# 42jaylonw/shifu

Hardware: AMD Instinct MI355X
Metric: env-steps/sec (whole node), A1 12-dof 4096 envs/GPU (higher is better)
Workload: dtype f32

## Files before the change

### shifu_amd/csrc/shf_a1_chain.hip

```cpp
#include <hip/hip_runtime.h>

#include "shf_chain.h"
#include "shf_chain_hard.h"

template <int G, bool TW, bool SELF = false>
__global__ __launch_bounds__(256, (G == 32 ? 2 : 1)) void k_a1_chain(A1Args A) { a1_chain_step_body<G, A1Chain, TW, SELF>(A); }

template <bool TW, bool SELF>
__global__ __launch_bounds__(256, 2) void k_a1_chain_pgs(A1Args A) { a1_chain_step_body<32, A1Chain, TW, SELF, true>(A); }
template <bool TW, bool SELF>
__global__ __launch_bounds__(256, 2) void k_a1_chain_pgs16(A1Args A) { a1_chain_step_body<32, A1Chain, TW, SELF, true, 16>(A); }
template <bool TW, bool SELF>
__global__ __launch_bounds__(256, 2) void k_a1_chain_tgs(A1Args A) { a1_chain_step_body<32, A1Chain, TW, SELF, true, 8, true>(A); }
template <bool TW, bool SELF>
__global__ __launch_bounds__(256, 2) void k_a1_chain_tgs16(A1Args A) { a1_chain_step_body<32, A1Chain, TW, SELF, true, 16, true>(A); }
#define SHF_PICK4(K, warped, self) ((self) ? ((warped) ? reinterpret_cast<const void*>(K<true, true>) : reinterpret_cast<const void*>(K<false, true>)) \
                                           : ((warped) ? reinterpret_cast<const void*>(K<true, false>) : reinterpret_cast<const void*>(K<false, false>)))
const void* shf_a1_chain_pgs_kernel(bool warped, bool self, bool k16, bool tgs) {
  if (tgs) return k16 ? SHF_PICK4(k_a1_chain_tgs16, warped, self) : SHF_PICK4(k_a1_chain_tgs, warped, self);
  return k16 ? SHF_PICK4(k_a1_chain_pgs16, warped, self) : SHF_PICK4(k_a1_chain_pgs, warped, self);
}
int shf_a1_chain_pgs_max_contacts(void) { return 16; }

template <bool TW, bool SELF, int KC, bool TGS>
DEV void sim_step_chain_pgs_body(const SimArgs& A) {
  extern __shared__ __attribute__((aligned(16))) float smem[];
  typedef A1Chain CD;
  constexpr int G = 32, nb = CD::NB, nd = CD::ND, NR = (CD::NEV + G - 1) / G;
  const int es = threadIdx.x / G, l = threadIdx.x % G;
  const int e = blockIdx.x * (256 / G) + es;
  stage_block<CHAIN_MODEL_BYTES>(A.model, smem);
  __syncthreads();
  const ShfModel* m = reinterpret_cast<const ShfModel*>(smem);
  if (e >= A.n) return;
  ChainLds L = chain_lds_carve<CD>(smem + CHAIN_MODEL_WORDS + es * chain_lds_words<CD>(0, SELF));
  const float* dof = A.dof + (size_t)e * nd * 2;
  const float* root = A.root + (size_t)e * 13;
  for (int i = l; i < 2 * nd; i += G) L.dofb[(i >> 1) * DOF_STRIDE + (i & 1)] = dof[i];
  if (l < 13) L.root[l] = root[l];
  GROUP_SYNC();
  StepCtx C;
  C.m = m; C.sp = A.sp; C.terr.t = A.terr; C.terr.h = A.heights; C.scene = nullptr;
  C.dropped = env_dropped(A.dropped, A.sp, e);
  C.mscale = A.mscale ? A.mscale + (size_t)e * nb : nullptr;
  const float mu = A.friction ? A.friction[e] : 1.0f;
  const int dl = l < nd ? l : 0;
  DofLane X = {L.dofb[dl * DOF_STRIDE], L.dofb[dl * DOF_STRIDE + 1], (A.effort && l < nd) ? A.effort[(size_t)e * nd + l] : 0.0f,
               (A.pos_tgt && l < nd) ? A.pos_tgt[(size_t)e * nd + l] : 0.0f, (A.vel_tgt && l < nd) ? A.vel_tgt[(size_t)e * nd + l] : 0.0f};
  ChainPoints<NR> LP;
  chain_points_load<G>(m, CD::NEV, l, C.sp.contact_offset + C.sp.rest_offset, LP);
  const RowLane RL = row_lane_load<CD>(l);
  chain_substep_hard<G, CD, TW, SELF, KC, TGS>(C, L, l, X, LP, RL, A.body_force ? A.body_force + (size_t)e * nb * 3 : nullptr, mu, L.xch);
  if (l < nd) {
    A.dof[((size_t)e * nd + l) * 2] = X.q;
    A.dof[((size_t)e * nd + l) * 2 + 1] = X.qd;
  }
  if (l < 13) A.root[(size_t)e * 13 + l] = L.root[l];
  for (int i = l; i < 3 * nb; i += G) A.contact[(size_t)e * nb * 3 + i] = L.xch[i];
}
template <bool TW, bool SELF>
__global__ __launch_bounds__(256, 2) void k_sim_step_chain_pgs(SimArgs A) { sim_step_chain_pgs_body<TW, SELF, 8, false>(A); }
template <bool TW, bool SELF>
__global__ __launch_bounds__(256, 2) void k_sim_step_chain_pgs16(SimArgs A) { sim_step_chain_pgs_body<TW, SELF, 16, false>(A); }
template <bool TW, bool SELF>
__global__ __launch_bounds__(256, 2) void k_sim_step_chain_tgs(SimArgs A) { sim_step_chain_pgs_body<TW, SELF, 8, true>(A); }
template <bool TW, bool SELF>
__global__ __launch_bounds__(256, 2) void k_sim_step_chain_tgs16(SimArgs A) { sim_step_chain_pgs_body<TW, SELF, 16, true>(A); }
const void* shf_sim_step_chain_pgs_kernel(bool warped, bool self, bool k16, bool tgs) {
  if (tgs) return k16 ? SHF_PICK4(k_sim_step_chain_tgs16, warped, self) : SHF_PICK4(k_sim_step_chain_tgs, warped, self);
  return k16 ? SHF_PICK4(k_sim_step_chain_pgs16, warped, self) : SHF_PICK4(k_sim_step_chain_pgs, warped, self);
}
size_t shf_sim_step_chain_pgs_lds_bytes(bool self) { return ((size_t)CHAIN_MODEL_WORDS + 8 * (size_t)chain_lds_words<A1Chain>(0, self)) * 4; }

bool shf_a1_chain_matches(const ShfModel& m) { return A1Chain::matches(m); }
size_t shf_a1_chain_lds_bytes(int G, int nobs, bool self) {
  const int epb = 256 / G;
  return ((size_t)CHAIN_MODEL_WORDS + TASK_WORDS + STATS_LDS_WORDS + (size_t)epb * chain_lds_words<A1Chain>(SCR_OBS + nobs, self)) * 4;
}
const void* shf_a1_chain_kernel(int G, bool warped, bool self) {
  if (self) {
    if (G != 32) return nullptr;
    return warped ? reinterpret_cast<const void*>(k_a1_chain<32, true, true>) : reinterpret_cast<const void*>(k_a1_chain<32, false, true>);
  }
  switch (G) {
    case 16: return warped ? reinterpret_cast<const void*>(k_a1_chain<16, true>) : reinterpret_cast<const void*>(k_a1_chain<16, false>);
    case 32: return warped ? reinterpret_cast<const void*>(k_a1_chain<32, true>) : reinterpret_cast<const void*>(k_a1_chain<32, false>);
    default: return nullptr;
  }
}
#ifdef SHF_PHASE_CLOCK
int shf_a1_chain_phase_cycles(unsigned long long* out, int n, int reset) {
  unsigned long long h[48];
  if (hipMemcpyFromSymbol(h, HIP_SYMBOL(g_phase_cycles), sizeof h) != hipSuccess) return 1;
  for (int k = 0; k < n && k < 48; k++) out[k] = h[k];
  if (reset) {
    unsigned long long z[48] = {};
    if (hipMemcpyToSymbol(HIP_SYMBOL(g_phase_cycles), z, sizeof z) != hipSuccess) return 1;
  }
  return 0;
}
#endif
```

### shifu_amd/csrc/shf_chain.h

```cpp
#pragma once
#include "shf_task.h"
#include "shf_link.h"

template <int NCH_, int NLK_, int NP_, int NEV_>
struct ChainDims {
  static constexpr int NCH = NCH_, NLK = NLK_, NB = 1 + NCH_ * (NLK_ + 1), ND = NCH_ * NLK_, NPC = NP_;
  static constexpr int NEV = NEV_;
  static constexpr int MAXPT = 9;
  static_assert(NEV_ >= NP_ && NEV_ <= 128, "evaluation slots: two 64-bit ballot words");
  DEV static constexpr int body(int c, int k) { return 1 + c * (NLK_ + 1) + k; }
  static bool matches(const ShfModel& m) {
    if (m.nb != NB || m.nd != ND || m.np != NPC || m.fixed_base || m.jtype[0] != SHF_JOINT_ROOT) return false;
    if (m.child_count[0] != NCH || m.nlevels != NLK) return false;
    if ((m.neval > 0 ? m.neval : m.np) != NEV) return false;
    int occupied = 0;
    for (int s = 0; s < NEV; s++) {
      const int i = m.pt_eval[s];
      if (i == -1) continue;
      if (i < 0 || i >= NPC || m.pt_slot[i] != s) return false;
      occupied++;
    }
    if (occupied != NPC) return false;
    for (int b = 0; b < NB; b++) {
      const int n = m.pt_count[b], i0 = m.pt_start[b];
// ... 649 lines not shown
    float* rec = L.jrec + l * JREC_STRIDE;
    float Rl[9];
    joint_local_rotation(m->trot[b], m->axis[b], X.q, Rl);
#pragma unroll
    for (int k = 0; k < 9; k++) rec[k] = Rl[k];
    rec[9] = X.qd;
  }
  GROUP_SYNC();
  if (l < NCH || l == ND) {
    float Rc[9], pc[3] = {0.0f, 0.0f, 0.0f}, vc[6], S[6], c[6];
    quat_to_mat(L.root + 3, Rc);
#pragma unroll
    for (int k = 0; k < 3; k++) { vc[k] = L.root[10 + k]; vc[3 + k] = L.root[7 + k]; }
    if (l == ND) {
      pose_store(L.pose, Rc, pc, vc);
    } else {
      const int b0 = CD::body(l, 0);
#pragma unroll
      for (int k = 0; k < NLK; k++) {
        const float* rec = L.jrec + (l * NLK + k) * JREC_STRIDE;
        float Rl[9];
#pragma unroll
        for (int j = 0; j < 9; j++) Rl[j] = rec[j];
        chain_compose_link(m->tpos[b0 + k], m->axis[b0 + k], Rl, rec[9], Rc, pc, vc, S, c);
        pose_store(L.pose + (b0 + k) * POSE_STRIDE, Rc, pc, vc);
      }
      chain_kin_weld(m->tpos[b0 + NLK], m->trot[b0 + NLK], Rc, pc);
      pose_store(L.pose + (b0 + NLK) * POSE_STRIDE, Rc, pc, vc);
    }
  }
  GROUP_SYNC();
  for (int b = l; b < NB; b += G) {
    const float* pb = L.pose + b * POSE_STRIDE;
    float Rw[9], pp[3], v[6], t[3], q[4];
#pragma unroll
    for (int k = 0; k < 9; k++) Rw[k] = pb[k];
#pragma unroll
    for (int k = 0; k < 3; k++) pp[k] = pb[9 + k];
#pragma unroll
    for (int k = 0; k < 6; k++) v[k] = pb[12 + k];
    float* o = stage + 13 * b;
#pragma unroll
    for (int k = 0; k < 3; k++) o[k] = L.root[k] + pp[k];
    mat_to_quat(Rw, q);
#pragma unroll
    for (int k = 0; k < 4; k++) o[3 + k] = q[k];
    cross3(v, pp, t);
#pragma unroll
    for (int k = 0; k < 3; k++) { o[7 + k] = v[3 + k] + t[k]; o[10 + k] = v[k]; }
  }
  GROUP_SYNC();
}

template <int G, class CD, bool TW, bool SELF, int KC, bool TGS>
DEV void chain_substep_hard(const StepCtx& C, const ChainLds& L, int l, DofLane& X, const ChainPoints<(CD::NEV + G - 1) / G>& P,
                            const RowLane& RL, const float* fext, float mu_shape, float* contact_out);
template <int G, class CD, bool TW, bool SELF = false, bool HARD = false, int KC = 8, bool TGS = false>
DEV void a1_chain_step_body(const A1Args& A) {
  extern __shared__ __attribute__((aligned(16))) float smem[];
  constexpr int NLK = CD::NLK, nb = CD::NB, nd = CD::ND, NR = (CD::NEV + G - 1) / G;
  PHASE_BEGIN();
  float* stats_lds = smem + CHAIN_MODEL_WORDS + TASK_WORDS;
  stats_block_init(stats_lds);
  const unsigned long long stats_step = stats_step_load(A.stats);
  const int epb = 256 / G, es = threadIdx.x / G, l = threadIdx.x % G;
  const int e = blockIdx.x * epb + es;
  const int n = A.S.n;
  constexpr int NW = (2 * nd + G - 1) / G;
  float pre_dof[NW], pre_root = 0.0f, pre_act = 0.0f;
#pragma unroll
  for (int k = 0; k < NW; k++) pre_dof[k] = 0.0f;
  static_assert(G >= 13 && G > nd, "one root word and one action per lane");
  if (e < n) {
#pragma unroll
    for (int k = 0; k < NW; k++)
      if (l + k * G < 2 * nd) pre_dof[k] = A.S.dof[(size_t)e * nd * 2 + l + k * G];
    if (l < 13) pre_root = A.S.root[(size_t)e * 13 + l];
    if (l < nd) pre_act = raw_action(A, e, l, nd, stats_step);
  }
  stage_block<(int)sizeof(ShfA1TaskParams)>(A.tp, smem + CHAIN_MODEL_WORDS);
  stage_block<CHAIN_MODEL_BYTES>(A.S.model, smem);
  __syncthreads();
  const ShfModel* m = reinterpret_cast<const ShfModel*>(smem);
  const ShfA1TaskParams& tp = *reinterpret_cast<const ShfA1TaskParams*>(smem + CHAIN_MODEL_WORDS);
  if (e >= n) return;
  const int H = tp.num_history, P = tp.num_height_points;
  const int nobs = 12 + 2 * nd + nd * H + P;
  const int env_words = chain_lds_words<CD>(SCR_OBS + nobs, SELF);
  ChainLds L = chain_lds_carve<CD>(smem + CHAIN_MODEL_WORDS + TASK_WORDS + STATS_LDS_WORDS + es * env_words);
  float* scr = L.pt;

#pragma unroll
  for (int k = 0; k < NW; k++) {
    const int i = l + k * G;
    if (i < 2 * nd) L.dofb[(i >> 1) * DOF_STRIDE + (i & 1)] = pre_dof[k];
  }
  if (l < 13) L.root[l] = pre_root;
  float act = 0.0f;
  if (l < nd) {
    act = rclampf(pre_act * tp.action_scale, -tp.clip_actions, tp.clip_actions);
    A.actions[(size_t)e * nd + l] = act;
  }
  GROUP_SYNC();

  if (l == 0) {
    const float gv[3] = {0.0f, 0.0f, -1.0f};
    float pg[3], blv[3], bav[3];
    quat_rotate_inverse(L.root + 3, L.root + 7, blv);
    quat_rotate_inverse(L.root + 3, L.root + 10, bav);
    quat_rotate_inverse(L.root + 3, gv, pg);
    float* o = A.base_vel + (size_t)e * 9;
#pragma unroll
    for (int k = 0; k < 3; k++) { o[k] = blv[k]; o[3 + k] = bav[k]; o[6 + k] = pg[k]; }
  }

  StepCtx C;
  C.m = m; C.sp = A.S.sp; C.terr.t = A.S.terr; C.terr.h = A.S.heights; C.scene = nullptr;
  if constexpr (HARD) C.dropped = env_dropped(A.S.dropped, A.S.sp, e);
  C.mscale = A.S.mscale ? A.S.mscale + (size_t)e * nb : nullptr;
  const float mu = A.S.friction[e];
  const int nsub = tp.decimation + (tp.extra_substep ? 1 : 0);
  const int dl = l < nd ? l : 0;
  DofLane X = {L.dofb[dl * DOF_STRIDE], L.dofb[dl * DOF_STRIDE + 1], 0.0f};
  const float pg_ = tp.p_gain[dl], dg_ = tp.d_gain[dl], q0_ = tp.default_dof_pos[dl], lim_ = m->effort[dl];
  ChainPoints<NR> LP;
  chain_points_load<G>(m, CD::NEV, l, HARD ? C.sp.contact_offset + C.sp.rest_offset : C.sp.contact_offset, LP);
  const int lb = G >= 32 ? (l & 15) : l;
  const int mb = lb < nd ? CD::body(lb / NLK, lb % NLK) : 0;
  const SlotList<CD::MAXPT> mine = slot_list_load<CD::MAXPT>(m, m->pt_start[mb], (lb <= nd && l < 32) ? m->pt_count[mb] : 0);
  const RowLane RL = row_lane_load<CD>(l);
  PHASE_MARK(11);
  for (int it = 0; it < nsub; it++) {
    if (it < tp.decimation) {
      const float t = pg_ * (act + q0_ - X.q) - dg_ * X.qd;
      X.tau = rclampf(t, -lim_, lim_);
    }
    if constexpr (HARD)
      chain_substep_hard<G, CD, TW, SELF, KC, TGS>(C, L, l, X, LP, RL, (it == tp.decimation) ? A.push + (size_t)e * nb * 3 : nullptr, mu,
                                    (it == nsub - 1) ? L.xch : nullptr);
    else
      chain_substep<G, CD, TW, SELF>(C, L, l, X, LP, mine, RL, (it == tp.decimation) ? A.push + (size_t)e * nb * 3 : nullptr, mu,
                                     (it == nsub - 1) ? L.xch : nullptr);
  }
  PHASE_RESET();
  if (l < nd) {
    float* D = L.dofb + l * DOF_STRIDE;
    D[0] = X.q; D[1] = X.qd; D[5] = X.tau;
    A.torques[(size_t)e * nd + l] = X.tau;
    scr[SCR_ACT + l] = act;
  }
  for (int i = l; i < 3 * nb; i += G) A.S.contact[(size_t)e * nb * 3 + i] = L.xch[i];
  for (int i = l; i < nd * H; i += G) scr[SCR_HIST + i] = A.history[(size_t)e * nd * H + i];
  PHASE_MARK(12);
  chain_body_states<G, CD>(m, L, l, X, scr + SCR_BODY);
  for (int i = l; i < 13 * nb; i += G) A.body_state[(size_t)e * nb * 13 + i] = scr[SCR_BODY + i];
  PHASE_RESET();
  a1_post_step<G>(A, m, tp, L, scr, e, l, stats_lds, stats_step);
}
```

### shifu_amd/csrc/shf_chain_hard.h

```cpp
#pragma once
#include "shf_chain.h"

#define UF_STRIDE 8
template <class CD, int KC>
struct HardTail {
  static constexpr int HC = 0, W = KC * HC_STRIDE, NEVP = (CD::NEV + 3) & ~3;
  static constexpr bool PACKED = KC > 8;
  static constexpr int WS = PACKED ? 9 : 10;
  static constexpr int NBLK = PACKED ? KC * (KC + 1) / 2 : KC * KC;
  static constexpr int NB0 = PACKED ? (CD::NPC * PT_STRIDE - W) / 9 : NBLK;
  static constexpr int UF = W, PHI = W, END = W + NB0 * WS;
  static constexpr int SPARE = CD::NB * POSE_STRIDE + ((CD::NB * 6 + 3) & ~3) + CD::ND * XCH_STRIDE;
  static_assert(NEVP + SHF_MAX_SELF_CONTACTS <= NB0 * WS && CD::ND * UF_STRIDE <= NB0 * WS, "the gap list / U, 1/D fit the response matrix's place");
  static_assert(!PACKED || (NBLK - NB0) * 9 <= SPARE, "the rest of the packed response matrix fits the pose / rate / exchange slots");
  static_assert(KC <= 16 && (W % 2) == 0, "owner lanes, 16-bit constraint masks; 8-byte aligned blocks");
};
template <class CD, int KC>
DEV float* hard_wblock(const ChainLds& L, float* tail, int i, int j) {
  typedef HardTail<CD, KC> T;
  if constexpr (T::PACKED) {
    const int b = ((j * (j + 1)) >> 1) + i;
    return b < T::NB0 ? tail + T::W + b * 9 : L.pose + (b - T::NB0) * 9;
  } else {
    return tail + T::W + (j * KC + i) * T::WS;
  }
}

DEV void mat3_inv_spd(const float* A, float* Ai) {
  const float c00 = fmaf(A[4], A[8], -(A[5] * A[7])), c01 = fmaf(A[5], A[6], -(A[3] * A[8])), c02 = fmaf(A[3], A[7], -(A[4] * A[6]));
  const float id = rcp_spec(fmaf(A[0], c00, fmaf(A[1], c01, A[2] * c02)));
  Ai[0] = c00 * id; Ai[1] = fmaf(A[2], A[7], -(A[1] * A[8])) * id; Ai[2] = fmaf(A[1], A[5], -(A[2] * A[4])) * id;
  Ai[3] = c01 * id; Ai[4] = fmaf(A[0], A[8], -(A[2] * A[6])) * id; Ai[5] = fmaf(A[2], A[3], -(A[0] * A[5])) * id;
  Ai[6] = c02 * id; Ai[7] = fmaf(A[1], A[6], -(A[0] * A[7])) * id; Ai[8] = fmaf(A[0], A[4], -(A[1] * A[3])) * id;
}
#define LREC_U 6
#define LREC_INVD 12
struct HardLink { float S[6], U[6], invD; };
DEV HardLink hard_link_load(const float* rec) {
  const float4* r4 = reinterpret_cast<const float4*>(rec);
  const float4 a = r4[0], b = r4[1], c = r4[2], d = r4[3];
  HardLink K;
  K.S[0] = a.x; K.S[1] = a.y; K.S[2] = a.z; K.S[3] = a.w; K.S[4] = b.x; K.S[5] = b.y;
  K.U[0] = b.z; K.U[1] = b.w; K.U[2] = c.x; K.U[3] = c.y; K.U[4] = c.z; K.U[5] = c.w;
  K.invD = d.x;
  return K;
}
template <class CD>
struct HardResp { int cs, ks; float ub[CD::NLK], dv0[6]; };
template <class CD>
DEV void hard_impulse(const ChainLds& L, const float* tail, int bs, const float* r, const float* e, HardResp<CD>& q) {
  constexpr int NLK = CD::NLK;
  q.cs = bs > 0 ? (bs - 1) / (NLK + 1) : 0;
  q.ks = bs > 0 ? (bs - 1) % (NLK + 1) : -1;
  float p6[6], t[3];
  cross3(r, e, t);
#pragma unroll
  for (int k = 0; k < 3; k++) { p6[k] = -t[k]; p6[3 + k] = -e[k]; }
#pragma unroll
  for (int k = NLK - 1; k >= 0; k--) {
    q.ub[k] = 0.0f;
    if (k <= q.ks) {
      const HardLink Lk = hard_link_load(L.jrec + (q.cs * NLK + k) * JREC_STRIDE);
      float sp = Lk.S[0] * p6[0];
#pragma unroll
      for (int j = 1; j < 6; j++) sp = fmaf(Lk.S[j], p6[j], sp);
      q.ub[k] = -sp;
      const float tt = q.ub[k] * Lk.invD;
#pragma unroll
      for (int j = 0; j < 6; j++) p6[j] = fmaf(Lk.U[j], tt, p6[j]);
    }
  }
  root_factors_apply(L.xroot, p6, q.dv0);
}
template <class CD>
DEV void hard_velocity(const ChainLds& L, const float* tail, const HardResp<CD>& q, int bt, const float* r, float* vel) {
  constexpr int NLK = CD::NLK;
  if (bt < 0) { vel[0] = 0.0f; vel[1] = 0.0f; vel[2] = 0.0f; return; }
  const int ct = bt > 0 ? (bt - 1) / (NLK + 1) : 0, kt = bt > 0 ? (bt - 1) % (NLK + 1) : -1;
  float dv[6];
#pragma unroll
  for (int j = 0; j < 6; j++) dv[j] = q.dv0[j];
#pragma unroll
  for (int k = 0; k < NLK; k++) {
    if (k <= kt) {
      const HardLink Lk = hard_link_load(L.jrec + (ct * NLK + k) * JREC_STRIDE);
      const float ubk = (ct == q.cs && k <= q.ks) ? q.ub[k] : 0.0f;
      float ua = Lk.U[0] * dv[0];
#pragma unroll
      for (int j = 1; j < 6; j++) ua = fmaf(Lk.U[j], dv[j], ua);
      const float dq = (ubk - ua) * Lk.invD;
#pragma unroll
      for (int j = 0; j < 6; j++) dv[j] = fmaf(Lk.S[j], dq, dv[j]);
    }
  }
  hard_point(dv, r, vel);
}

template <class CD, int NQ, int KC>
DEV void chain_hard_apply(const ShfModel* m, const ChainLds& L, float* tail, int l, int K, float idt, bool isbody_h0, bool islink, bool isroot,
                          bool ischain, int ci, int lb, int myb, float (*ac0)[6]) {
  constexpr int NCH = CD::NCH, NLK = CD::NLK;
  typedef HardTail<CD, KC> T;
  float pcr[NQ][6];
#pragma unroll
  for (int q = 0; q < NQ; q++)
#pragma unroll
    for (int j = 0; j < 6; j++) pcr[q][j] = 0.0f;
  if (isbody_h0) {
    unsigned mine_a = 0u, mine_b = 0u;
#pragma unroll
    for (int c = 0; c < KC; c++) {
      const float* h = tail + T::HC + c * HC_STRIDE;
      const int ia = __float_as_int(h[HC_BODY]), ib = __float_as_int(h[HC_BODYB]);
      if (c < K && ia == myb) mine_a |= 1u << c;
      if (c < K && ib == myb) mine_b |= 1u << c;
    }
    for (unsigned bits = mine_a | mine_b; bits; bits &= bits - 1u) {
      const int c = __builtin_ctz(bits);
      const float* h = tail + T::HC + c * HC_STRIDE;
      const bool ona = (mine_a >> c) & 1u;
      const float r[3] = {h[HC_R], h[HC_R + 1], h[HC_R + 2]};
#pragma unroll
      for (int q = 0; q < NQ; q++) {
        const float f[3] = {h[q == 0 ? HC_P : HC_PV0] * idt, h[q == 0 ? HC_P + 1 : HC_PV1] * idt, h[q == 0 ? HC_P + 2 : HC_PV2] * idt};
        float t[3];
        cross3(r, f, t);
        if (ona) {
#pragma unroll
          for (int k = 0; k < 3; k++) { pcr[q][k] -= t[k]; pcr[q][3 + k] -= f[k]; }
        } else {
#pragma unroll
          for (int k = 0; k < 3; k++) { pcr[q][k] += t[k]; pcr[q][3 + k] += f[k]; }
        }
      }
    }
    if (islink) {
      float* o = L.xch + lb * XCH_STRIDE;
#pragma unroll
      for (int q = 0; q < NQ; q++)
#pragma unroll
        for (int j = 0; j < 6; j++) o[(q == 0 ? 21 : 8) + j] = pcr[q][j];
    }
  }
  GROUP_SYNC();
  float ucl[NQ][NLK];
  if (ischain) {
    float pl[NQ][6];
#pragma unroll
    for (int k = NLK - 1; k >= 0; k--) {
      const int li = ci * NLK + k;
// ... 19 lines not shown
        for (int j = 0; j < 6; j++) pl[q][j] = fmaf(U[j], tt, pl[q][j]);
      }
    }
    float* o = L.xch + (ci * NLK) * XCH_STRIDE;
#pragma unroll
    for (int q = 0; q < NQ; q++)
#pragma unroll
      for (int j = 0; j < 6; j++) o[(q == 0 ? 21 : 8) + j] = pl[q][j];
  }
  GROUP_SYNC();
  if (isroot) {
#pragma unroll
    for (int q = 0; q < NQ; q++) {
#pragma unroll
      for (int j = 0; j < 6; j++) {
        float v = pcr[q][j];
#pragma unroll
        for (int c = 0; c < NCH; c++) v += L.xch[(c * NLK) * XCH_STRIDE + (q == 0 ? 21 : 8) + j];
        pcr[q][j] = v;
      }
      root_factors_apply(L.xroot, pcr[q], ac0[q]);
#pragma unroll
      for (int j = 0; j < 6; j++) L.acc[6 * q + j] = ac0[q][j];
    }
  }
  GROUP_SYNC();
  if (ischain) {
    float ac[NQ][6];
#pragma unroll
    for (int q = 0; q < NQ; q++)
#pragma unroll
      for (int j = 0; j < 6; j++) ac[q][j] = L.acc[6 * q + j];
#pragma unroll
    for (int k = 0; k < NLK; k++) {
      const int li = ci * NLK + k;
      const HardLink Lk = hard_link_load(L.jrec + li * JREC_STRIDE);
      const float* S = Lk.S; const float* U = Lk.U;
      const float invD = Lk.invD;
#pragma unroll
      for (int q = 0; q < NQ; q++) {
        float ua = U[0] * ac[q][0];
#pragma unroll
        for (int j = 1; j < 6; j++) ua = fmaf(U[j], ac[q][j], ua);
        const float qc = (ucl[q][k] - ua) * invD;
#pragma unroll
        for (int j = 0; j < 6; j++) ac[q][j] = fmaf(S[j], qc, ac[q][j]);
        L.dofb[li * DOF_STRIDE + 2 + q] = qc;
      }
    }
  }
  GROUP_SYNC();
}

template <int G, class CD, bool TW, bool SELF, int KC, bool TGS>
DEV void chain_substep_hard(const StepCtx& C, const ChainLds& L, int l, DofLane& X, const ChainPoints<(CD::NEV + G - 1) / G>& P,
                            const RowLane& RL, const float* fext, float mu_shape, float* contact_out) {
  static_assert(G == 32, "the velocity-level solve is written for two envs per wavefront");
  constexpr int NCH = CD::NCH, NLK = CD::NLK, NB = CD::NB, ND = CD::ND, NR = (CD::NEV + G - 1) / G;
  typedef HardTail<CD, KC> T;
  static_assert(T::END <= CD::NPC * PT_STRIDE, "the solve's LDS fits the contact-slot region");
  static_assert((KC == 8 || KC == 16) && KC <= G / 2 + 8 && ND < 16, "owner lanes; a lane per column of the response matrix, in one or two passes");
  const ShfModel* m = C.m;
  const float dt = C.sp.dt, idt = 1.0f / dt;
  const float gon = (float)m->gravity_on;
  const float g[3] = {C.sp.gravity[0] * gon, C.sp.gravity[1] * gon, C.sp.gravity[2] * gon};
  float* tail = L.pt;
  const int lb = l & 15;
  const int half = (l >> 4) & 1;
  const bool isdof = l < ND, isroot = l == ND;
  const bool ischain = (l & 7) == 0 && (l >> 3) < NCH;
  const int ci = l >> 3;
  const bool isbody = lb <= ND;
  const bool islink = isbody && lb < ND;
  const int myb = lb < ND ? CD::body(lb / NLK, lb % NLK) : 0;
  const int lane0 = (int)(threadIdx.x & 63u) - l;
  PHASE_BEGIN();

  if (isdof) {
    float* rec = L.jrec + l * JREC_STRIDE;
    float Rl[9], t0, de;
    chain_dof_effort(C, l, X.q, X.qd, X.tau, &t0, &de, X.tq, X.tv);
    joint_local_rotation(m->trot[myb], m->axis[myb], X.q, Rl);
#pragma unroll
    for (int k = 0; k < 9; k++) rec[k] = Rl[k];
    rec[JREC_QD] = X.qd; rec[JREC_T0] = t0; rec[JREC_DE] = de;
  }
  GROUP_SYNC();
  PHASE_MARK(0);

  if (ischain || isroot) {
    float Rc[9], pc[3] = {0.0f, 0.0f, 0.0f}, vc[6];
    quat_to_mat(L.root + 3, Rc);
#pragma unroll
    for (int k = 0; k < 3; k++) { vc[k] = L.root[10 + k]; vc[3 + k] = L.root[7 + k]; }
    if (isroot && !ischain) {
      pose_store(L.pose, Rc, pc, vc);
    } else {
      const int b0 = CD::body(ci, 0);
#pragma unroll
      for (int k = 0; k < NLK; k++) {
        const int b = b0 + k;
        float* rec = L.jrec + (ci * NLK + k) * JREC_STRIDE;
        float Rl[9], Sx[6], cx[6];
#pragma unroll
        for (int j = 0; j < 9; j++) Rl[j] = rec[j];
        chain_compose_link(m->tpos[b], m->axis[b], Rl, rec[JREC_QD], Rc, pc, vc, Sx, cx);
#pragma unroll
        for (int j = 0; j < 6; j++) { rec[JREC_S + j] = Sx[j]; rec[JREC_C + j] = cx[j]; }
        pose_store(L.pose + b * POSE_STRIDE, Rc, pc, vc);
      }
      const int b = b0 + NLK;
      chain_kin_weld(m->tpos[b], m->trot[b], Rc, pc);
      pose_store(L.pose + b * POSE_STRIDE, Rc, pc, vc);
    }
  }
  GROUP_SYNC();
  PHASE_MARK(1);

  if (isbody) {
    float IA[21], pA[6];
    const float* pb = L.pose + myb * POSE_STRIDE;
    float Rb[9], pp[3], vb[6];
#pragma unroll
    for (int k = 0; k < 9; k++) Rb[k] = pb[k];
#pragma unroll
    for (int k = 0; k < 3; k++) pp[k] = pb[9 + k];
#pragma unroll
    for (int k = 0; k < 6; k++) vb[k] = pb[12 + k];
    {
// ... 299 lines not shown
      const float* h = tail + T::HC + (own ? l : 0) * HC_STRIDE;
      const float r[3] = {h[HC_R], h[HC_R + 1], h[HC_R + 2]};
      const float n[3] = {h[HC_N], h[HC_N + 1], h[HC_N + 2]};
#pragma unroll
      for (int k = 0; k < 3; k++) O.p[k] = 0.0f;
      O.mu = h[HC_MU];
      const int b = own ? __float_as_int(h[HC_BODY]) : 0;
      const float* pb = L.pose + b * POSE_STRIDE + 12;
      const float* D = L.acc + b * 6;
      float v[6], v6[6], vs[3], vf[3], vsb[3] = {0.0f, 0.0f, 0.0f}, vfb[3] = {0.0f, 0.0f, 0.0f};
#pragma unroll
      for (int k = 0; k < 6; k++) { v[k] = pb[k]; v6[k] = fmaf(dt, D[k], v[k]); }
      hard_point(v, r, vs);
      hard_point(v6, r, vf);
      if constexpr (SELF) {
        const int b2 = own ? __float_as_int(h[HC_BODYB]) : -1;
        if (b2 >= 0) {
          const float* pb2 = L.pose + b2 * POSE_STRIDE + 12;
          const float* D2 = L.acc + b2 * 6;
#pragma unroll
          for (int k = 0; k < 6; k++) { v[k] = pb2[k]; v6[k] = fmaf(dt, D2[k], v[k]); }
          hard_point(v, r, vsb);
          hard_point(v6, r, vfb);
        }
      }
#pragma unroll
      for (int k = 0; k < 3; k++) { vf[k] = vf[k] - vfb[k]; vs[k] = vs[k] - vsb[k]; }
      O.u[0] = dot3(n, vf); O.u[1] = dot3(h + HC_T1, vf); O.u[2] = dot3(h + HC_T2, vf);
      const float phi = h[HC_PHI];
      const float erp = C.sp.erp > 0.0f ? C.sp.erp : 0.2f;
      float tg = phi >= 0.0f ? -(phi * idt) : rminf(erp * -(phi) * idt, C.sp.max_depen_vel);
      float tv = phi >= 0.0f ? tg : 0.0f;
      const float vn0 = dot3(n, vs);
      if (C.sp.restitution > 0.0f && vn0 < -C.sp.bounce_threshold) { tg = rmaxf(tg, -(C.sp.restitution * vn0)); tv = rmaxf(tv, -(C.sp.restitution * vn0)); }
      O.tgt = tg; O.tgt_v = tv;
      O.gap = phi;
      O.rfloor = (C.sp.restitution > 0.0f && vn0 < -C.sp.bounce_threshold) ? -(C.sp.restitution * vn0) : -1e30f;
    };
    if constexpr (T::PACKED) owner_velocities();
    if constexpr (T::PACKED) GROUP_SYNC();
#pragma unroll 1
    for (int q0 = 0; q0 < 3 * KC; q0 += G) {
      const int q = q0 + l;
      if (__ballot(q < 3 * K) == 0ull) break;
      const int j = (q * 43) >> 7, ax = q - 3 * j;
      const bool col = q < 3 * K;
      const float* hj = tail + T::HC + (col ? j : 0) * HC_STRIDE;
      const float rj[3] = {hj[HC_R], hj[HC_R + 1], hj[HC_R + 2]};
      const int bsa = col ? __float_as_int(hj[HC_BODY]) : 0;
      const int bsb = (SELF && col) ? __float_as_int(hj[HC_BODYB]) : -1;
      const float* ej = hj + (ax == 0 ? HC_N : (ax == 1 ? HC_T1 : HC_T2));
      const float e[3] = {ej[0], ej[1], ej[2]};
      HardResp<CD> qa, qb;
      hard_impulse<CD>(L, tail, bsa, rj, e, qa);
      if constexpr (SELF) {
        if (__ballot(bsb >= 0) != 0ull) hard_impulse<CD>(L, tail, bsb >= 0 ? bsb : 0, rj, e, qb);
      }
#pragma unroll 1
      for (int d = 0; 2 * d <= KC; d++) {
        if (__ballot(2 * d <= K) == 0ull) break;
        const bool todo = col && 2 * d <= K && d < K && !(d > 0 && 2 * d == K && 2 * j < K);
        int i = j - d;
        if (i < 0) i += K;
        if (!todo) continue;
        const float* hi = tail + T::HC + i * HC_STRIDE;
        const float ri[3] = {hi[HC_R], hi[HC_R + 1], hi[HC_R + 2]};
        const int bta = __float_as_int(hi[HC_BODY]);
        float aa[3], ab[3] = {0.0f, 0.0f, 0.0f}, ba[3] = {0.0f, 0.0f, 0.0f}, bb[3] = {0.0f, 0.0f, 0.0f};
        hard_velocity<CD>(L, tail, qa, bta, ri, aa);
        if constexpr (SELF) {
          const int btb = __float_as_int(hi[HC_BODYB]);
          hard_velocity<CD>(L, tail, qa, btb, ri, ab);
          if (bsb >= 0) {
            hard_velocity<CD>(L, tail, qb, bta, ri, ba);
            hard_velocity<CD>(L, tail, qb, btb, ri, bb);
          }
        }
        float vw[3];
#pragma unroll
        for (int r = 0; r < 3; r++) vw[r] = (aa[r] - ab[r]) - (ba[r] - bb[r]);
        const float w0 = dot3(hi + HC_N, vw), w1 = dot3(hi + HC_T1, vw), w2 = dot3(hi + HC_T2, vw);
        if constexpr (T::PACKED) {
          if (i <= j) { float* Wb = hard_wblock<CD, KC>(L, tail, i, j) + ax; Wb[0] = w0; Wb[3] = w1; Wb[6] = w2; }
          else { float* Wt = hard_wblock<CD, KC>(L, tail, j, i) + 3 * ax; Wt[0] = w0; Wt[1] = w1; Wt[2] = w2; }
        } else {
          float* Wb = hard_wblock<CD, KC>(L, tail, i, j) + ax;
          Wb[0] = w0; Wb[3] = w1; Wb[6] = w2;
          if (i != j) { float* Wt = hard_wblock<CD, KC>(L, tail, j, i) + 3 * ax; Wt[0] = w0; Wt[1] = w1; Wt[2] = w2; }
        }
      }
    }
    GROUP_SYNC();
    PHASE_MARK(5);

    if constexpr (!T::PACKED) owner_velocities();
    {
      float* Wd = hard_wblock<CD, KC>(L, tail, own ? l : 0, own ? l : 0);
      float A[9];
#pragma unroll
      for (int k = 0; k < 9; k++) A[k] = Wd[k];
      const float cfm = 1e-6f * ((A[0] + A[4]) + A[8]);
      A[0] += cfm; A[4] += cfm; A[8] += cfm;
      const float s01 = 0.5f * (A[1] + A[3]), s02 = 0.5f * (A[2] + A[6]), s12 = 0.5f * (A[5] + A[7]);
      A[1] = s01; A[3] = s01; A[2] = s02; A[6] = s02; A[5] = s12; A[7] = s12;
      if (own) {
#pragma unroll
        for (int k = 0; k < 9; k++) Wd[k] = A[k];
      }
      O.iwnn = rcp_spec(A[0]);
      O.w10 = A[3]; O.w20 = A[6];
      const float id = rcp_spec(fmaf(A[4], A[8], -(A[5] * A[5])));
      O.Ti[0] = A[8] * id; O.Ti[1] = -(A[5] * id); O.Ti[2] = A[4] * id;
      O.rt = rcp_spec(A[4] + A[8]);
    }
    GROUP_SYNC();
    PHASE_MARK(10);

    int Kw = 0;
#pragma unroll
    for (int c = 0; c < KC; c++)
      if (__ballot(c < K) != 0ull) Kw = c + 1;
    const bool hi = lane0 != 0;
#ifdef SHF_PHASE_CLOCK
    if ((threadIdx.x & 63u) == 0u) atomicAdd(&g_phase_cycles[38 + (Kw < 8 ? Kw : 8)], 1ull);
#endif
    const float* Wcol = tail + T::W + (own ? l : 0) * T::WS;
    const int li = own ? l : 0;
    auto wload8 = [&](int c, float* Wb) {
      const float2* b2 = reinterpret_cast<const float2*>(Wcol + c * KC * T::WS);
      const float2 w01 = b2[0], w23 = b2[1], w45 = b2[2], w67 = b2[3];
      Wb[0] = w01.x; Wb[1] = w01.y; Wb[2] = w23.x; Wb[3] = w23.y; Wb[4] = w45.x; Wb[5] = w45.y; Wb[6] = w67.x; Wb[7] = w67.y;
      Wb[8] = Wcol[c * KC * T::WS + 8];
    };
    const unsigned long long ownm = __ballot(own);
    auto visit8 = [&](auto cc, float tg, const float* Wb) {
      constexpr int c = decltype(cc)::value;
      constexpr unsigned long long lanes_c = (1ull << c) | (1ull << (32 + c));
      const unsigned long long act = __ballot(O.p[0] != 0.0f) | __ballot(O.p[1] != 0.0f) | __ballot(O.p[2] != 0.0f) | __ballot(O.u[0] < tg);
      const unsigned long long cm = act & ownm & lanes_c;
      if (cm == 0ull) return;
      const bool commit = __builtin_amdgcn_inverse_ballot_w64(cm);
      const float pn0 = O.p[0];
      const float pn = rmaxf(fmaf(-(O.u[0] - tg), O.iwnn, pn0), 0.0f);
      const float dn = pn - pn0;
      const float ut1 = fmaf(dn, O.w10, O.u[1]), ut2 = fmaf(dn, O.w20, O.u[2]);
      float ps1 = O.p[1] - fmaf(O.Ti[1], ut2, O.Ti[0] * ut1), ps2 = O.p[2] - fmaf(O.Ti[2], ut2, O.Ti[1] * ut1);
      const float lim = O.mu * pn, lim2 = lim * lim;
      const bool slide = fmaf(ps2, ps2, ps1 * ps1) > lim2;
      if ((cm & __ballot(slide)) != 0ull) {
        float q1 = fmaf(-O.rt, ut1, O.p[1]), q2 = fmaf(-O.rt, ut2, O.p[2]);
        const float nt2 = fmaf(q2, q2, q1 * q1);
        const float sc1 = nt2 > rmaxf(lim2, 1e-30f) ? lim * rsqrt_spec(nt2) : 1.0f;
        q1 *= sc1; q2 *= sc1;
        ps1 = slide ? q1 : ps1; ps2 = slide ? q2 : ps2;
      }
      const float n0 = commit ? pn : O.p[0], n1 = commit ? ps1 : O.p[1], n2 = commit ? ps2 : O.p[2];
      const float dp0 = n0 - O.p[0], dp1 = n1 - O.p[1], dp2 = n2 - O.p[2];
      O.p[0] = n0; O.p[1] = n1; O.p[2] = n2;
      const float b0 = hard_row_bcast<c>(dp0), b1 = hard_row_bcast<c>(dp1), b2 = hard_row_bcast<c>(dp2);
      const bool take = own && c < K;
#pragma unroll
      for (int r = 0; r < 3; r++) {
        const float ur = fmaf(Wb[3 * r + 2], b2, fmaf(Wb[3 * r + 1], b1, fmaf(Wb[3 * r], b0, O.u[r])));
        O.u[r] = take ? ur : O.u[r];
      }
    };
    auto visit = [&](int c, float tg) {
      const bool act = !(O.p[0] == 0.0f && O.p[1] == 0.0f && O.p[2] == 0.0f && !(O.u[0] < tg));
      if (__ballot(l == c && c < K && act) == 0ull) return;
      float Wb[9];
      {
        const bool tr = li > c;
        const float* blk = hard_wblock<CD, KC>(L, tail, tr ? c : li, tr ? li : c);
        float Ws[9];
#pragma unroll
        for (int k = 0; k < 9; k++) Ws[k] = blk[k];
#pragma unroll
        for (int r = 0; r < 3; r++)
#pragma unroll
          for (int k = 0; k < 3; k++) Wb[3 * r + k] = tr ? Ws[3 * k + r] : Ws[3 * r + k];
      }
      const float pn0 = O.p[0];
      const float pn = rmaxf(fmaf(-(O.u[0] - tg), O.iwnn, pn0), 0.0f);
      const float dn = pn - pn0;
      const float ut1 = fmaf(dn, O.w10, O.u[1]), ut2 = fmaf(dn, O.w20, O.u[2]);
      float ps1 = O.p[1] - fmaf(O.Ti[1], ut2, O.Ti[0] * ut1), ps2 = O.p[2] - fmaf(O.Ti[2], ut2, O.Ti[1] * ut1);
      const float lim = O.mu * pn, lim2 = lim * lim;
      const bool commit = l == c && c < K && act;
      if (commit && fmaf(ps2, ps2, ps1 * ps1) > lim2) {
        ps1 = fmaf(-O.rt, ut1, O.p[1]); ps2 = fmaf(-O.rt, ut2, O.p[2]);
        const float nt2 = fmaf(ps2, ps2, ps1 * ps1);
        const float sc1 = nt2 > rmaxf(lim2, 1e-30f) ? lim * rsqrt_spec(nt2) : 1.0f;
        ps1 *= sc1; ps2 *= sc1;
      }
      const float n0 = commit ? pn : O.p[0], n1 = commit ? ps1 : O.p[1], n2 = commit ? ps2 : O.p[2];
      float dp0 = n0 - O.p[0], dp1 = n1 - O.p[1], dp2 = n2 - O.p[2];
      O.p[0] = n0; O.p[1] = n1; O.p[2] = n2;
      {
        const float a0 = hard_readlane(dp0, c), a1 = hard_readlane(dp1, c), a2 = hard_readlane(dp2, c);
        const float b0 = hard_readlane(dp0, 32 + c), b1 = hard_readlane(dp1, 32 + c), b2 = hard_readlane(dp2, 32 + c);
        dp0 = hi ? b0 : a0; dp1 = hi ? b1 : a1; dp2 = hi ? b2 : a2;
      }
      if (own && c < K) {
#pragma unroll
        for (int r = 0; r < 3; r++) O.u[r] = fmaf(Wb[3 * r + 2], dp2, fmaf(Wb[3 * r + 1], dp1, fmaf(Wb[3 * r], dp0, O.u[r])));
      }
    };
    const HardTgs TG = hard_tgs(C.sp, npos);
    float psum[3] = {0.0f, 0.0f, 0.0f};
#pragma unroll 1
    for (int phase = 0; phase < 2; phase++) {
      const int sweeps = phase == 0 ? npos : nvel;
      float tg = phase == 0 ? O.tgt : O.tgt_v;
      if constexpr (TGS) { if (phase == 1) tg = hard_tgs_target_vel(TG, O); }
#pragma unroll 1
      for (int it = 0; it < sweeps; it++) {
        if constexpr (TGS) { if (phase == 0) tg = hard_tgs_target_pos(TG, O); }
        if constexpr (T::PACKED) {
#pragma unroll 1
          for (int c = 0; c < Kw; c++) visit(c, tg);
        } else {
          float Wb[KC][9];
          wload8(0, Wb[0]);
          hard_static_while<0, KC>([&](auto cc) {
            constexpr int c = decltype(cc)::value;
            if (c >= Kw) return false;
            if constexpr (c + 1 < KC) wload8(c + 1, Wb[c + 1]);
            visit8(cc, tg, Wb[c]);
            return true;
          });
        }
        if constexpr (TGS) {
          if (phase == 0) {
            O.gap = fmaf(TG.hN, O.u[0], O.gap);
#pragma unroll
            for (int r = 0; r < 3; r++) psum[r] += O.p[r];
          }
        }
      }
      if (phase == 1 && nvel == 0) break;
      if (own) {
        float* h = tail + T::HC + l * HC_STRIDE;
        float pw[3];
        const bool mean = TGS && phase == 0;
        const float q0 = mean ? psum[0] * TG.inv_n : O.p[0], q1 = mean ? psum[1] * TG.inv_n : O.p[1], q2 = mean ? psum[2] * TG.inv_n : O.p[2];
#pragma unroll
        for (int r = 0; r < 3; r++) pw[r] = fmaf(q2, h[HC_T2 + r], fmaf(q1, h[HC_T1 + r], q0 * h[HC_N + r]));
        if (phase == 0) { h[HC_P] = pw[0]; h[HC_P + 1] = pw[1]; h[HC_P + 2] = pw[2]; }
        else { h[HC_PV0] = pw[0]; h[HC_PV1] = pw[1]; h[HC_PV2] = pw[2]; }
      }
    }
    PHASE_MARK(17);
    GROUP_SYNC();
    if (nvel > 0) chain_hard_apply<CD, 2, KC>(m, L, tail, l, K, idt, isbody && half == 0, islink, isroot, ischain, ci, lb, myb, ac0);
    else chain_hard_apply<CD, 1, KC>(m, L, tail, l, K, idt, isbody && half == 0, islink, isroot, ischain, ci, lb, myb, ac0);
    PHASE_MARK(18);
  } else {
    if (isdof) { L.dofb[l * DOF_STRIDE + 2] = 0.0f; L.dofb[l * DOF_STRIDE + 3] = 0.0f; }
  }
  PHASE_MARK(4);

  if (isdof) {
    const float vl = m->vel_limit[l];
    const float qf = L.dofb[l * DOF_STRIDE + 4];
    const float qcp = K > 0 ? L.dofb[l * DOF_STRIDE + 2] : 0.0f;
    const float qcv = K > 0 ? (nvel > 0 ? L.dofb[l * DOF_STRIDE + 3] : qcp) : 0.0f;
    const float qdv = K > 0 ? qf + qcv : qf, qdp = K > 0 ? qf + qcp : qf;
    const float qdn = rclampf(fmaf(dt, qdv, X.qd), -vl, vl);
    const float qpn = rclampf(fmaf(dt, qdp, X.qd), -vl, vl);
    X.q = fmaf(dt, qpn, X.q);
    X.qd = qdn;
  }
  if (isroot) {
    float av[6], apz[6];
#pragma unroll
    for (int j = 0; j < 6; j++) {
      const float cv = nvel > 0 ? ac0[1][j] : ac0[0][j];
      av[j] = K > 0 ? a0[j] + cv : a0[j];
      apz[j] = K > 0 ? a0[j] + ac0[0][j] : a0[j];
    }
    float* Rt = L.root;
// ... 59 lines not shown
```

Baseline: 23.60 million.

## Keep W response rows in registers and batch link loads in hard contact solve

For the KC=8 PGS/TGS kernels, the per-owner rows of the contact response matrix W are loaded into registers once before the sweep loops instead of being reloaded from LDS on every sweep. Building W now preloads each chain's link records in one batch and prefetches the next target record, so fewer LDS reads sit on the critical path. Contact point loading is moved inside the substep so its registers are live only there. This raises register pressure, with a risk of spilling or lower occupancy under launch_bounds(256,2).

New measurement: 24.54 million, median of 6. +4.0%, better.

```diff
diff --git a/shifu_amd/csrc/shf_a1_chain.hip b/shifu_amd/csrc/shf_a1_chain.hip
--- a/shifu_amd/csrc/shf_a1_chain.hip
+++ b/shifu_amd/csrc/shf_a1_chain.hip
@@ -6,12 +6,18 @@
 template <int G, bool TW, bool SELF = false>
 __global__ __launch_bounds__(256, (G == 32 ? 2 : 1)) void k_a1_chain(A1Args A) { a1_chain_step_body<G, A1Chain, TW, SELF>(A); }
 
+#ifndef SHF_WR_FUSED
+#define SHF_WR_FUSED 8
+#endif
+#ifndef SHF_WR_HOOK
+#define SHF_WR_HOOK 0
+#endif
 template <bool TW, bool SELF>
-__global__ __launch_bounds__(256, 2) void k_a1_chain_pgs(A1Args A) { a1_chain_step_body<32, A1Chain, TW, SELF, true>(A); }
+__global__ __launch_bounds__(256, 2) void k_a1_chain_pgs(A1Args A) { a1_chain_step_body<32, A1Chain, TW, SELF, true, 8, false, SHF_WR_FUSED>(A); }
 template <bool TW, bool SELF>
 __global__ __launch_bounds__(256, 2) void k_a1_chain_pgs16(A1Args A) { a1_chain_step_body<32, A1Chain, TW, SELF, true, 16>(A); }
 template <bool TW, bool SELF>
-__global__ __launch_bounds__(256, 2) void k_a1_chain_tgs(A1Args A) { a1_chain_step_body<32, A1Chain, TW, SELF, true, 8, true>(A); }
+__global__ __launch_bounds__(256, 2) void k_a1_chain_tgs(A1Args A) { a1_chain_step_body<32, A1Chain, TW, SELF, true, 8, true, SHF_WR_FUSED>(A); }
 template <bool TW, bool SELF>
 __global__ __launch_bounds__(256, 2) void k_a1_chain_tgs16(A1Args A) { a1_chain_step_body<32, A1Chain, TW, SELF, true, 16, true>(A); }
 #define SHF_PICK4(K, warped, self) ((self) ? ((warped) ? reinterpret_cast<const void*>(K<true, true>) : reinterpret_cast<const void*>(K<false, true>)) \
@@ -50,7 +56,7 @@
   ChainPoints<NR> LP;
   chain_points_load<G>(m, CD::NEV, l, C.sp.contact_offset + C.sp.rest_offset, LP);
   const RowLane RL = row_lane_load<CD>(l);
-  chain_substep_hard<G, CD, TW, SELF, KC, TGS>(C, L, l, X, LP, RL, A.body_force ? A.body_force + (size_t)e * nb * 3 : nullptr, mu, L.xch);
+  chain_substep_hard<G, CD, TW, SELF, KC, TGS, (KC == 8 ? SHF_WR_HOOK : 0)>(C, L, l, X, LP, RL, A.body_force ? A.body_force + (size_t)e * nb * 3 : nullptr, mu, L.xch);
   if (l < nd) {
     A.dof[((size_t)e * nd + l) * 2] = X.q;
     A.dof[((size_t)e * nd + l) * 2 + 1] = X.qd;
diff --git a/shifu_amd/csrc/shf_chain.h b/shifu_amd/csrc/shf_chain.h
--- a/shifu_amd/csrc/shf_chain.h
+++ b/shifu_amd/csrc/shf_chain.h
@@ -725,10 +725,10 @@
   GROUP_SYNC();
 }
 
-template <int G, class CD, bool TW, bool SELF, int KC, bool TGS>
+template <int G, class CD, bool TW, bool SELF, int KC, bool TGS, int WR>
 DEV void chain_substep_hard(const StepCtx& C, const ChainLds& L, int l, DofLane& X, const ChainPoints<(CD::NEV + G - 1) / G>& P,
                             const RowLane& RL, const float* fext, float mu_shape, float* contact_out);
-template <int G, class CD, bool TW, bool SELF = false, bool HARD = false, int KC = 8, bool TGS = false>
+template <int G, class CD, bool TW, bool SELF = false, bool HARD = false, int KC = 8, bool TGS = false, int WR = 0>
 DEV void a1_chain_step_body(const A1Args& A) {
   extern __shared__ __attribute__((aligned(16))) float smem[];
   constexpr int NLK = CD::NLK, nb = CD::NB, nd = CD::ND, NR = (CD::NEV + G - 1) / G;
@@ -797,7 +797,7 @@
   DofLane X = {L.dofb[dl * DOF_STRIDE], L.dofb[dl * DOF_STRIDE + 1], 0.0f};
   const float pg_ = tp.p_gain[dl], dg_ = tp.d_gain[dl], q0_ = tp.default_dof_pos[dl], lim_ = m->effort[dl];
   ChainPoints<NR> LP;
-  chain_points_load<G>(m, CD::NEV, l, HARD ? C.sp.contact_offset + C.sp.rest_offset : C.sp.contact_offset, LP);
+  if constexpr (!(HARD && WR > 0)) chain_points_load<G>(m, CD::NEV, l, HARD ? C.sp.contact_offset + C.sp.rest_offset : C.sp.contact_offset, LP);
   const int lb = G >= 32 ? (l & 15) : l;
   const int mb = lb < nd ? CD::body(lb / NLK, lb % NLK) : 0;
   const SlotList<CD::MAXPT> mine = slot_list_load<CD::MAXPT>(m, m->pt_start[mb], (lb <= nd && l < 32) ? m->pt_count[mb] : 0);
@@ -809,7 +809,7 @@
       X.tau = rclampf(t, -lim_, lim_);
     }
     if constexpr (HARD)
-      chain_substep_hard<G, CD, TW, SELF, KC, TGS>(C, L, l, X, LP, RL, (it == tp.decimation) ? A.push + (size_t)e * nb * 3 : nullptr, mu,
+      chain_substep_hard<G, CD, TW, SELF, KC, TGS, WR>(C, L, l, X, LP, RL, (it == tp.decimation) ? A.push + (size_t)e * nb * 3 : nullptr, mu,
                                     (it == nsub - 1) ? L.xch : nullptr);
     else
       chain_substep<G, CD, TW, SELF>(C, L, l, X, LP, mine, RL, (it == tp.decimation) ? A.push + (size_t)e * nb * 3 : nullptr, mu,
diff --git a/shifu_amd/csrc/shf_chain_hard.h b/shifu_amd/csrc/shf_chain_hard.h
--- a/shifu_amd/csrc/shf_chain_hard.h
+++ b/shifu_amd/csrc/shf_chain_hard.h
@@ -48,10 +48,19 @@
 template <class CD>
 struct HardResp { int cs, ks; float ub[CD::NLK], dv0[6]; };
 template <class CD>
+DEV void hard_links_load(const ChainLds& L, int b, HardLink* Lk) {
+  constexpr int NLK = CD::NLK;
+  const int c = b > 0 ? (b - 1) / (NLK + 1) : 0;
+#pragma unroll
+  for (int k = 0; k < NLK; k++) Lk[k] = hard_link_load(L.jrec + (c * NLK + k) * JREC_STRIDE);
+}
+template <class CD, bool BATCH = false>
 DEV void hard_impulse(const ChainLds& L, const float* tail, int bs, const float* r, const float* e, HardResp<CD>& q) {
   constexpr int NLK = CD::NLK;
   q.cs = bs > 0 ? (bs - 1) / (NLK + 1) : 0;
   q.ks = bs > 0 ? (bs - 1) % (NLK + 1) : -1;
+  HardLink Lb[NLK];
+  if constexpr (BATCH) hard_links_load<CD>(L, bs, Lb);
   float p6[6], t[3];
   cross3(r, e, t);
 #pragma unroll
@@ -60,7 +69,7 @@
   for (int k = NLK - 1; k >= 0; k--) {
     q.ub[k] = 0.0f;
     if (k <= q.ks) {
-      const HardLink Lk = hard_link_load(L.jrec + (q.cs * NLK + k) * JREC_STRIDE);
+      const HardLink Lk = BATCH ? Lb[k] : hard_link_load(L.jrec + (q.cs * NLK + k) * JREC_STRIDE);
       float sp = Lk.S[0] * p6[0];
 #pragma unroll
       for (int j = 1; j < 6; j++) sp = fmaf(Lk.S[j], p6[j], sp);
@@ -96,6 +105,38 @@
   hard_point(dv, r, vel);
 }
 
+template <class CD>
+DEV void hard_velocity_links(const HardResp<CD>& q, int bt, const HardLink* Lc, const float* r, float* vel) {
+  constexpr int NLK = CD::NLK;
+  if (bt < 0) { vel[0] = 0.0f; vel[1] = 0.0f; vel[2] = 0.0f; return; }
+  const int ct = bt > 0 ? (bt - 1) / (NLK + 1) : 0, kt = bt > 0 ? (bt - 1) % (NLK + 1) : -1;
+  float dv[6];
+#pragma unroll
+  for (int j = 0; j < 6; j++) dv[j] = q.dv0[j];
+#pragma unroll
+  for (int k = 0; k < NLK; k++) {
+    if (k <= kt) {
+      const HardLink& Lk = Lc[k];
+      const float ubk = (ct == q.cs && k <= q.ks) ? q.ub[k] : 0.0f;
+      float ua = Lk.U[0] * dv[0];
+#pragma unroll
+      for (int j = 1; j < 6; j++) ua = fmaf(Lk.U[j], dv[j], ua);
+      const float dq = (ubk - ua) * Lk.invD;
+#pragma unroll
+      for (int j = 0; j < 6; j++) dv[j] = fmaf(Lk.S[j], dq, dv[j]);
+    }
+  }
+  hard_point(dv, r, vel);
+}
+struct HardTarget { float r[3], n[3], t1[3], t2[3]; int ba; };
+DEV HardTarget hard_target_load(const float* h) {
+  HardTarget t;
+#pragma unroll
+  for (int k = 0; k < 3; k++) { t.r[k] = h[HC_R + k]; t.n[k] = h[HC_N + k]; t.t1[k] = h[HC_T1 + k]; t.t2[k] = h[HC_T2 + k]; }
+  t.ba = __float_as_int(h[HC_BODY]);
+  return t;
+}
+
 template <class CD, int NQ, int KC>
 DEV void chain_hard_apply(const ShfModel* m, const ChainLds& L, float* tail, int l, int K, float idt, bool isbody_h0, bool islink, bool isroot,
                           bool ischain, int ci, int lb, int myb, float (*ac0)[6]) {
@@ -221,14 +262,16 @@
   GROUP_SYNC();
 }
 
-template <int G, class CD, bool TW, bool SELF, int KC, bool TGS>
-DEV void chain_substep_hard(const StepCtx& C, const ChainLds& L, int l, DofLane& X, const ChainPoints<(CD::NEV + G - 1) / G>& P,
+template <int G, class CD, bool TW, bool SELF, int KC, bool TGS, int WR>
+DEV void chain_substep_hard(const StepCtx& C, const ChainLds& L, int l, DofLane& X, const ChainPoints<(CD::NEV + G - 1) / G>& PIN,
                             const RowLane& RL, const float* fext, float mu_shape, float* contact_out) {
   static_assert(G == 32, "the velocity-level solve is written for two envs per wavefront");
   constexpr int NCH = CD::NCH, NLK = CD::NLK, NB = CD::NB, ND = CD::ND, NR = (CD::NEV + G - 1) / G;
   typedef HardTail<CD, KC> T;
   static_assert(T::END <= CD::NPC * PT_STRIDE, "the solve's LDS fits the contact-slot region");
   static_assert((KC == 8 || KC == 16) && KC <= G / 2 + 8 && ND < 16, "owner lanes; a lane per column of the response matrix, in one or two passes");
+  static_assert(WR >= 0 && WR <= KC && (WR == 0 || !T::PACKED), "the register row is the KC = 8 layout's");
+  constexpr bool PIPE = WR > 0 && !SELF;
   const ShfModel* m = C.m;
   const float dt = C.sp.dt, idt = 1.0f / dt;
   const float gon = (float)m->gravity_on;
@@ -244,6 +287,9 @@
   const int myb = lb < ND ? CD::body(lb / NLK, lb % NLK) : 0;
   const int lane0 = (int)(threadIdx.x & 63u) - l;
   PHASE_BEGIN();
+  ChainPoints<NR> PL;
+  if constexpr (WR > 0) chain_points_load<G>(C.m, CD::NEV, l, C.sp.contact_offset + C.sp.rest_offset, PL);
+  const ChainPoints<NR>& P = WR > 0 ? PL : PIN;
 
   if (isdof) {
     float* rec = L.jrec + l * JREC_STRIDE;
@@ -649,10 +695,37 @@
       const float* ej = hj + (ax == 0 ? HC_N : (ax == 1 ? HC_T1 : HC_T2));
       const float e[3] = {ej[0], ej[1], ej[2]};
       HardResp<CD> qa, qb;
-      hard_impulse<CD>(L, tail, bsa, rj, e, qa);
+      hard_impulse<CD, PIPE>(L, tail, bsa, rj, e, qa);
       if constexpr (SELF) {
-        if (__ballot(bsb >= 0) != 0ull) hard_impulse<CD>(L, tail, bsb >= 0 ? bsb : 0, rj, e, qb);
-      }
+        if (__ballot(bsb >= 0) != 0ull) hard_impulse<CD, PIPE>(L, tail, bsb >= 0 ? bsb : 0, rj, e, qb);
+      }
+      if constexpr (PIPE) {
+        static_assert(!SELF && !T::PACKED, "one chain per target; W in full");
+        auto target_rec = [&](int d) {
+          int i = j - d;
+          if (i < 0) i += K;
+          return tail + T::HC + ((i >= 0 && i < KC) ? i : 0) * HC_STRIDE;
+        };
+        HardTarget nxt = hard_target_load(target_rec(0));
+#pragma unroll 1
+        for (int d = 0; 2 * d <= KC; d++) {
+          if (__ballot(2 * d <= K) == 0ull) break;
+          const bool todo = col && 2 * d <= K && d < K && !(d > 0 && 2 * d == K && 2 * j < K);
+          int i = j - d;
+          if (i < 0) i += K;
+          const HardTarget cur = nxt;
+          nxt = hard_target_load(target_rec(d + 1));
+          if (!todo) continue;
+          HardLink curL[NLK];
+          hard_links_load<CD>(L, cur.ba, curL);
+          float vw[3];
+          hard_velocity_links<CD>(qa, cur.ba, curL, cur.r, vw);
+          const float w0 = dot3(cur.n, vw), w1 = dot3(cur.t1, vw), w2 = dot3(cur.t2, vw);
+          float* Wb = hard_wblock<CD, KC>(L, tail, i, j) + ax;
+          Wb[0] = w0; Wb[3] = w1; Wb[6] = w2;
+          if (i != j) { float* Wt = hard_wblock<CD, KC>(L, tail, j, i) + 3 * ax; Wt[0] = w0; Wt[1] = w1; Wt[2] = w2; }
+        }
+      } else
 #pragma unroll 1
       for (int d = 0; 2 * d <= KC; d++) {
         if (__ballot(2 * d <= K) == 0ull) break;
@@ -729,6 +802,11 @@
       Wb[0] = w01.x; Wb[1] = w01.y; Wb[2] = w23.x; Wb[3] = w23.y; Wb[4] = w45.x; Wb[5] = w45.y; Wb[6] = w67.x; Wb[7] = w67.y;
       Wb[8] = Wcol[c * KC * T::WS + 8];
     };
+    float Wrow[WR > 0 ? WR : 1][9];
+    if constexpr (WR > 0) {
+#pragma unroll
+      for (int c = 0; c < WR; c++) wload8(c, Wrow[c]);
+    }
     const unsigned long long ownm = __ballot(own);
     auto visit8 = [&](auto cc, float tg, const float* Wb) {
       constexpr int c = decltype(cc)::value;
@@ -818,12 +896,12 @@
           for (int c = 0; c < Kw; c++) visit(c, tg);
         } else {
           float Wb[KC][9];
-          wload8(0, Wb[0]);
+          if constexpr (WR == 0) wload8(0, Wb[0]);
           hard_static_while<0, KC>([&](auto cc) {
             constexpr int c = decltype(cc)::value;
             if (c >= Kw) return false;
-            if constexpr (c + 1 < KC) wload8(c + 1, Wb[c + 1]);
-            visit8(cc, tg, Wb[c]);
+            if constexpr (c + 1 < KC && c + 1 >= WR) wload8(c + 1, Wb[c + 1]);
+            if constexpr (c < WR) visit8(cc, tg, Wrow[c]); else visit8(cc, tg, Wb[c]);
             return true;
           });
         }
```
